# vpecanins/stm32f7-rtlsdr

Measured on AMD Instinct MI355X. Metric: IQ MSamples/s through FIR+FM-demod+resample, higher is better.
Workload: dtype f32 audio; K2 = u8 x 24-bit fixed-point taps on the i8 matrix pipe, exact i32 sums, one f32 recombination (design Q); K3 / K4 f32; ill-conditioned phases recomputed with the f32 fmaf chain

## Files before the change

stm32f7-rtlsdr_amd/csrc/sdrfm_q.hip:

```cpp
#include <hip/hip_runtime.h>
#include <hip/hip_ext.h>

#include <cstddef>
#include <cstdint>
#include <type_traits>

#include "sdrfm_math.h"
#include "sdrfm_q.h"
#include "sdrfm_b.h"

typedef int qi4_t __attribute__((ext_vector_type(4)));
typedef int qi8_t __attribute__((ext_vector_type(8)));
typedef float qf2_t __attribute__((ext_vector_type(2)));
__device__ void q_raw_buffer_load_lds(qi4_t rsrc, __attribute__((address_space(3))) void* lds, int size, int voffset, int soffset,
                                      int offset, int aux) __asm("llvm.amdgcn.raw.buffer.load.lds");

namespace {

constexpr int QTA = (int)SDRFM_Q_TA;
constexpr int DB0 = 128;
constexpr int ABS = 4;
constexpr int ABW = 128 * ABS;
constexpr int FLW = 64 + 2;
#ifndef SDRFM_Q_GTAB
// ... 4 lines not shown
constexpr int QTP = (int)SDRFM_Q_TP;
template <int D, int DA>
struct QGeo {
  static constexpr int NCH = D / 2;
  static constexpr int NSC = (D + 3) / 4;
  static constexpr int BLKB = 16 * D;
  static constexpr int STEPB = 16 * BLKB;
  static constexpr int PRE = BLKB;
  static constexpr int DBW = DB0 + 128 * DA + 16;
  static constexpr int RWIN = QTP + 2 * D;
  static constexpr bool ALIGNED = (STEPB % 1024) == 0;
  static constexpr int CS = STEPB / 1024;
  static_assert(QTP % 4 == 0 && (2 * D) % 4 == 0, "the repair path loads whole groups of four samples, none of which straddles the call's first sample");
  static_assert(QTP + 2 * D <= 96, "the tap table of the repair path sits below the d history");
  static_assert(D % 2 == 0 && D <= 16 && (ALIGNED || D == 10), "geometries the ring logic is written for");
};
#ifndef SDRFM_Q_HO_RING
#define SDRFM_Q_HO_RING 1
#endif
#ifndef SDRFM_Q_K3
#define SDRFM_Q_K3 1
#endif
#ifndef SDRFM_Q_XORSKIP
#define SDRFM_Q_XORSKIP 1
#endif
#ifndef SDRFM_Q_PEEL
#define SDRFM_Q_PEEL 1
#endif
#ifndef SDRFM_Q_MICRO
#define SDRFM_Q_MICRO 1
#endif
#ifndef SDRFM_Q_AUX
#define SDRFM_Q_AUX 2
#endif
#ifndef SDRFM_Q_WQB
#define SDRFM_Q_WQB 4
#endif
constexpr int WQB = SDRFM_Q_WQB;
static_assert(WQB >= 4 && WQB <= 16 && 8 * WQB >= (int)SDRFM_Q_TA, "a warm-up holds the d history of a run's first audio output");

__device__ __forceinline__ float q_discriminate(float yr, float yi, float pr, float pi) {
  const float re = __builtin_fmaf(yr, pr, yi * pi);
  const float im = yi * pr - yr * pi;
  const float ax = __builtin_fabsf(re), ay = __builtin_fabsf(im);
  const float mx = __builtin_fmaxf(__builtin_fmaxf(ax, ay), 0x1p-120f), mn = __builtin_fminf(ax, ay);
  const float v = mn * __builtin_amdgcn_rcpf(mx);
  const float s2 = v * v;
  float q = 0x1.e34882p-8f;
  q = __builtin_fmaf(q, s2, -0x1.22fc74p-5f);
  q = __builtin_fmaf(q, s2, 0x1.509024p-4f);
  q = __builtin_fmaf(q, s2, -0x1.12688cp-3f);
  q = __builtin_fmaf(q, s2, 0x1.96c562p-3f);
  q = __builtin_fmaf(q, s2, -0x1.554086p-2f);
  float a = __builtin_fmaf(v, s2 * q, v);
  if (ay > ax) a = 0x1.921fb6p+0f - a;
  if (re < 0.0f) a = 0x1.921fb6p+1f - a;
  return __builtin_copysignf(a, im);
}

__device__ __forceinline__ float q_angle(float yr, float yi, float& mx_out) {
  const float ax = __builtin_fabsf(yr), ay = __builtin_fabsf(yi);
  const float mx = __builtin_fmaxf(__builtin_fmaxf(ax, ay), 0x1p-120f), mn = __builtin_fminf(ax, ay);
  mx_out = mx;
  const float v = mn * __builtin_amdgcn_rcpf(mx);
  const float s2 = v * v;
  float q = 0x1.e34882p-8f;
  q = __builtin_fmaf(q, s2, -0x1.22fc74p-5f);
  q = __builtin_fmaf(q, s2, 0x1.509024p-4f);
  q = __builtin_fmaf(q, s2, -0x1.12688cp-3f);
  q = __builtin_fmaf(q, s2, 0x1.96c562p-3f);
  q = __builtin_fmaf(q, s2, -0x1.554086p-2f);
  float a = __builtin_fmaf(v, s2 * q, v);
  if (ay > ax) a = 0x1.921fb6p+0f - a;
  if (yr < 0.0f) a = 0x1.921fb6p+1f - a;
  return __builtin_copysignf(a, yi);
}
__device__ __forceinline__ float q_wrap(float x) {
  float t = __builtin_fmaf(x, 0x1.45f306p-3f, 0x1.8p+23f);
  asm volatile("" : "+v"(t));
  const float k = t - 0x1.8p+23f;
  return __builtin_fmaf(k, -0x1.921fb6p+2f, x);
}

__device__ __forceinline__ unsigned q_pcm_word(float v) {
  const float c = __builtin_amdgcn_fmed3f(v, -32768.0f, 32767.0f);
  float t = c + 0x1.8p+23f;
  asm volatile("" : "+v"(t));
  return __builtin_amdgcn_perm(__builtin_bit_cast(unsigned, t), __builtin_bit_cast(unsigned, t), 0x05040504u);
}

template <int N>
__device__ __forceinline__ void wait_vmcnt() {
  static_assert(N >= 0 && N < 16, "vmcnt immediate");
  __builtin_amdgcn_s_waitcnt(0x0f70 | N);
}

#ifdef SDRFM_Q_PHASES
#define Q_PHASE(i) do { const unsigned long long tn_ = __builtin_readcyclecounter(); t_ph[i] += tn_ - t_last; t_last = tn_; } while (0)
#else
#define Q_PHASE(i) do { } while (0)
#endif

template <int D, int DA, int NSLOT>
constexpr uint32_t q_lds() { return (uint32_t)(QGeo<D, DA>::PRE + 1024 * NSLOT + 4 * (QGeo<D, DA>::DBW + ABW + FLW + GTW)); }
struct QPcmArgs { SdrfmQParams p; SdrfmSinkChain t; };
static_assert(ABS * 128 <= 64 * (int)SDRFM_CHAIN_CH, "a flush of parked audio is one scan of the wave");
template <int C0, int NSLOT, int D, int DA, bool PCM = false>
__device__ __forceinline__ void mfir_body(const SdrfmQParams& p, const uint32_t bid) {
  using G = QGeo<D, DA>;
  [[maybe_unused]] constexpr int NCH = G::NCH;
  constexpr int QD = D, QDA = DA, NSC = G::NSC, BLKB = G::BLKB, STEPB = G::STEPB, PRE = G::PRE, DBW = G::DBW, RWIN = G::RWIN;
  constexpr bool ALIGNED = G::ALIGNED;
  constexpr int CS = G::CS;
  constexpr int RINGB = NSLOT * 1024;
  static_assert(RINGB % (2 * STEPB) == 0 && (ALIGNED ? NSLOT == 2 * CS : (NSLOT >= 5 && NSLOT - 4 < 16)), "ring: whole pairs of steps");
  extern __shared__ __attribute__((aligned(16))) unsigned char smem[];
  float* const db = reinterpret_cast<float*>(smem + PRE + RINGB);
  float* const ab = db + DBW;
  unsigned short* const fl16 = reinterpret_cast<unsigned short*>(ab + ABW);
  const int lane = (int)threadIdx.x, n = lane & 15, g = lane >> 4;
  const uint32_t si = bid / p.runs, run = bid - si * p.runs;
  const uint32_t stream = p.slist ? p.slist[si] : si;
  const uint32_t Bt = (p.M + 7u) >> 3, Qt = (Bt + WQB - 1u) / WQB, vs = p.iq_prev ? 1u : 0u;
  const uint32_t Gq = Qt + p.runs - 1u + vs;
  const uint32_t e0 = (uint32_t)(((uint64_t)run * Gq) / p.runs), e1 = (uint32_t)(((uint64_t)(run + 1) * Gq) / p.runs);
  const int q0 = run == 0 ? 0 : (int)e0 - (int)(run - 1u + vs), q1 = (int)e1 - (int)(run + vs);
  if (q0 >= q1) return;
  if (lane == 0) *reinterpret_cast<uint2*>(fl16 + 128) = make_uint2(0u, 0u);
#ifdef SDRFM_Q_STAMPS
  unsigned long long* const tsp = p.dbg ? p.dbg + 16 * (size_t)bid : nullptr;
  unsigned long long t_wait = 0, t_first = 0;
  const unsigned long long t_entry = __builtin_amdgcn_s_memrealtime();
  const unsigned long long c_entry = __builtin_readcyclecounter();
#endif
#ifdef SDRFM_Q_PHASES
  unsigned long long t_ph[8] = {0, 0, 0, 0, 0, 0, 0, 0}, t_last = 0;
#endif
  const bool from_prev = run == 0 && p.iq_prev != nullptr;
  const bool warm = run > 0 || from_prev;
  const int b0 = WQB * q0;
  int b1 = WQB * q1;
  if (b1 > (int)Bt) b1 = (int)Bt;
  const bool last_run = b1 == (int)Bt;
  const int bs = warm ? b0 - WQB : b0;
  const int nsteps = (b1 - bs + 15) >> 4;
  const int nlast = b1 - bs - 16 * (nsteps - 1);
  const int o0 = 8 * bs;
  const int jg0 = (o0 + 64 * QDA) / QDA - 64;
  const int jlo = warm ? (o0 + 8 * WQB) / QDA : 0;
  int j1 = (8 * b1) / QDA;
  if (j1 > (int)p.A_out) j1 = (int)p.A_out;
  const int phi = QDA * jg0 + QDA - 1 - o0;
  const int sigma = (phi + 1) & 1;

  float cr = 1.0e4f, ci = 0.0f;
  const int HT = (int)p.T - 1;
  unsigned short hb0 = 0, hb1 = 0;
  float hd0 = 0.0f;
  if (!warm) {
    const float2 yp = p.yprev_in[stream];
    cr = yp.x; ci = yp.y;
    const unsigned short* hbp = reinterpret_cast<const unsigned short*>(p.hist_b_in) + (size_t)stream * HT;
    if (lane < HT) hb0 = hbp[lane];
    if (lane + 64 < HT) hb1 = hbp[lane + 64];
    if (lane < QTA - 1) hd0 = p.hist_d_in[(size_t)stream * (QTA - 1) + lane];
  }

  const unsigned long long gaddr = (unsigned long long)(p.iq + (size_t)stream * p.iq_stride);
  uint32_t hi = (uint32_t)BLKB * (uint32_t)b1;
  if (hi > 2u * p.N) hi = 2u * p.N;
  const qi4_t rsrc = {(int)(unsigned)gaddr, (int)(unsigned)(gaddr >> 32), (int)hi, 0x00020000};
  const int lsw0 = ALIGNED ? ((16 * lane) ^ (((((16 * lane) / BLKB)) & 7) << 4)) : 16 * lane;
  const int lsw1 = ALIGNED ? ((16 * lane) ^ (((((1024 + 16 * lane) / BLKB)) & 7) << 4)) : 16 * lane;
  const int gb = BLKB * bs;
  int vpos = gb + (ALIGNED ? 0 : 16 * lane);
  auto slot_ptr = [&](int slot) { return (__attribute__((address_space(3))) void*)(smem + PRE + 1024 * slot); };
  auto lsw = [&](int chunk) { return (BLKB == 256 && (chunk & 1)) ? lsw1 : lsw0; };
  constexpr int HL = BLKB / 16, HK = ALIGNED ? 7 : 0;
  const unsigned long long pa = from_prev ? (unsigned long long)(p.iq_prev + (size_t)stream * p.iq_prev_stride) + 2ull * p.N_prev - (WQB + 1) * BLKB : 0ull;
  const qi4_t rprev = {(int)(unsigned)pa, (int)(unsigned)(pa >> 32), (WQB + 1) * BLKB, 0x00020000};
  if (warm && lane < HL) {
    const int hv = 16 * (lane ^ HK);
    if (from_prev) q_raw_buffer_load_lds(rprev, (__attribute__((address_space(3))) void*)smem, 16, hv, 0, 0, SDRFM_Q_AUX);
    else q_raw_buffer_load_lds(rsrc, (__attribute__((address_space(3))) void*)smem, 16, gb - BLKB + hv, 0, 0, SDRFM_Q_AUX);
  }
  if constexpr (ALIGNED) {
#pragma unroll
    for (int q = 0; q < CS; ++q) {
      const int off = gb + 1024 * q + lsw(q);
      if (from_prev && off < 0) q_raw_buffer_load_lds(rprev, slot_ptr(q), 16, off + (WQB + 1) * BLKB, 0, 0, SDRFM_Q_AUX);
      else q_raw_buffer_load_lds(rsrc, slot_ptr(q), 16, off, 0, 0, SDRFM_Q_AUX);
    }
  } else {
    auto first_step_chunk = [&](int c, __attribute__((address_space(3))) void* lds, int imm) {
      const int off = vpos + 1024 * c;
      if (from_prev && off < 0) q_raw_buffer_load_lds(rprev, lds, 16, off - imm + (WQB + 1) * BLKB, 0, imm, SDRFM_Q_AUX);
      else q_raw_buffer_load_lds(rsrc, lds, 16, off - imm, 0, imm, SDRFM_Q_AUX);
    };
    first_step_chunk(0, slot_ptr(0), 0);
    first_step_chunk(1, slot_ptr(1), 0);
    first_step_chunk(2, slot_ptr(0), 2048);
  }
  __builtin_amdgcn_sched_barrier(0);
  asm volatile("" ::: "memory");
  qi4_t At[NSC - C0][SDRFM_Q_DIGITS];
#pragma unroll
  for (int c = C0; c < NSC; ++c)
#pragma unroll
    for (int t = 0; t < SDRFM_Q_DIGITS; ++t)
#if defined(SDRFM_Q_ABLATE) && (SDRFM_Q_ABLATE & 4)
      At[c - C0][t] = qi4_t{lane + c, lane * t, c - t, lane};
// ... 77 lines not shown
    const unsigned long long tw0 = __builtin_readcyclecounter();
#endif
#ifdef SDRFM_Q_FIRSTWAIT
    if (!ALIGNED && first) wait_vmcnt<(ALIGNED ? CS : NSLOT - 3)>();
    else
#endif
    wait_vmcnt<(ALIGNED ? CS : NSLOT - 4)>();
    asm volatile("" ::: "memory");
#ifdef SDRFM_Q_LDSXOR
#pragma unroll
    for (int i = 0; i < STEPB / 512; ++i)
      (void)__hip_atomic_fetch_xor(reinterpret_cast<unsigned long long*>(__builtin_assume_aligned(smem + PRE + ringoff + 8 * (lane + 64 * i), 8)), 0x8080808080808080ull, __ATOMIC_RELAXED, __HIP_MEMORY_SCOPE_WAVEFRONT);
#endif
#ifdef SDRFM_Q_STAMPS
    t_wait += __builtin_readcyclecounter() - tw0;
    if (t_first == 0) t_first = __builtin_amdgcn_s_memrealtime();
#endif
    if constexpr (ALIGNED) {
      const int ro0 = n == 0 ? 0 : ringoff;
#pragma unroll
      for (int c = 2 * C0; c < 2 * NSC; ++c) dst[c - 2 * C0] = *reinterpret_cast<const qi4_t*>(smem + rdoff[c] + (64 * c < BLKB ? ro0 : ringoff));
      if (lane < BLKB / 16) {
        const qi4_t hcp = *reinterpret_cast<const qi4_t*>(smem + PRE + ringoff + STEPB - BLKB + 16 * lane);
        *reinterpret_cast<qi4_t*>(smem + 16 * lane) = hcp;
      }
      __builtin_amdgcn_wave_barrier();
    } else {
      const unsigned char* wb = smem + baddr + ringoff;
#pragma unroll
      for (int c = 2 * C0; c < 2 * NSC; ++c) dst[c - 2 * C0] = *reinterpret_cast<const qi4_t*>(wb + 64 * c);
      if (ringoff + STEPB == RINGB) {
        if (lane < BLKB / 16) {
          const qi4_t hcp = *reinterpret_cast<const qi4_t*>(smem + PRE + RINGB - BLKB + 16 * lane);
          *reinterpret_cast<qi4_t*>(smem + 16 * lane) = hcp;
        }
        __builtin_amdgcn_wave_barrier();
      }
    }
    if constexpr (RINGB == 2 * STEPB) ringoff ^= STEPB;
    else ringoff = (ringoff + STEPB == RINGB) ? 0 : ringoff + STEPB;
  };
  auto refill_step = [&](int k) {
    asm volatile("s_waitcnt lgkmcnt(0)" ::: "memory");
    if constexpr (ALIGNED) {
#pragma unroll
      for (int q = 0; q < CS; ++q) q_raw_buffer_load_lds(rsrc, slot_ptr(slot + q), 16, vpos + 1024 * q + lsw(q), 0, 0, SDRFM_Q_AUX);
      slot = slot ? 0 : CS;
      vpos += STEPB;
      return;
    }
    if constexpr (NSLOT == 5 && SDRFM_Q_PEEL) {
      if (k & 1) {
        q_raw_buffer_load_lds(rsrc, slot_ptr(2), 16, vpos, 0, 0, SDRFM_Q_AUX);
        q_raw_buffer_load_lds(rsrc, slot_ptr(2), 16, vpos, 0, 1024, SDRFM_Q_AUX);
        vpos += 2048;
      } else {
        if (k > 0) {
          q_raw_buffer_load_lds(rsrc, slot_ptr(4), 16, vpos, 0, 0, SDRFM_Q_AUX);
          vpos += 1024;
        }
        q_raw_buffer_load_lds(rsrc, slot_ptr(0), 16, vpos, 0, 0, SDRFM_Q_AUX);
        q_raw_buffer_load_lds(rsrc, slot_ptr(0), 16, vpos, 0, 1024, SDRFM_Q_AUX);
        vpos += 2048;
      }
      return;
    }
    if (k > 0 && !(k & 1)) {
      q_raw_buffer_load_lds(rsrc, slot_ptr(slot), 16, vpos, 0, 0, SDRFM_Q_AUX);
      vpos += 1024;
      slot = (slot + 1 == NSLOT) ? 0 : slot + 1;
    }
    q_raw_buffer_load_lds(rsrc, slot_ptr(slot), 16, vpos, 0, 0, SDRFM_Q_AUX);
    q_raw_buffer_load_lds(rsrc, slot_ptr(slot), 16, vpos, 0, 1024, SDRFM_Q_AUX);
    slot = (slot + 2 >= NSLOT) ? slot + 2 - NSLOT : slot + 2;
    vpos += 2048;
  };
  typedef const __attribute__((address_space(4))) SdrfmQParams* KargPtr;
  auto kargs = [&]() -> KargPtr {
    KargPtr pp = (KargPtr)__builtin_amdgcn_kernarg_segment_ptr();
    asm volatile("" : "+s"(pp));
    return pp;
  };
  int npend = 0, jfl = jg0;
  [[maybe_unused]] float yrun = 0.0f;
  [[maybe_unused]] bool pfirst = true;
  [[maybe_unused]] float* const pstash = reinterpret_cast<float*>(smem + q_lds<D, DA, NSLOT>());
  typedef const __attribute__((address_space(4))) SdrfmSinkChain* KChainPtr;
  [[maybe_unused]] auto kchain = [&]() -> KChainPtr {
    const __attribute__((address_space(4))) unsigned char* pp = (const __attribute__((address_space(4))) unsigned char*)__builtin_amdgcn_kernarg_segment_ptr();
    asm volatile("" : "+s"(pp));
    return (KChainPtr)(pp + offsetof(QPcmArgs, t));
  };
  [[maybe_unused]] unsigned long long pv_early = 0ull;
  [[maybe_unused]] bool published = false;
  [[maybe_unused]] float dp_early = 0.0f;
  auto flush_audio = [&](const bool fin = false) {
    __builtin_amdgcn_wave_barrier();
#if defined(SDRFM_Q_ABLATE) && (SDRFM_Q_ABLATE & 256)
    float* row = p.audio - jfl;
    const int ln_ = lane;
#else
    uint32_t st_ = stream;
    int ln_ = lane;
    asm volatile("" : "+s"(st_), "+v"(ln_));
    float* row = kargs()->audio + (size_t)st_ * kargs()->audio_stride;
#endif
    const int lo = jfl > jlo ? jfl : jlo;
#if defined(SDRFM_Q_ABLATE) && (SDRFM_Q_ABLATE & 128)
    const int hi_ = (ab[lane] == 1234.5f) ? lo + 2 : lo;
#else
    const int hi_ = (j1 < jfl + 128 * npend) ? j1 : jfl + 128 * npend;
#endif
    const int par = (int)((reinterpret_cast<uintptr_t>(row) >> 2) & 1u);
    bool want_audio = true;
    if constexpr (PCM) want_audio = kargs()->audio != nullptr;
    if (want_audio) for (int e = lo - ((lo + par) & 1) + 2 * ln_; e < hi_; e += 128) {
      const bool v0 = e >= lo, v1 = e + 1 < hi_;
      const float a0 = v0 ? ab[e - jfl] : 0.0f, a1 = v1 ? ab[e + 1 - jfl] : 0.0f;
      if constexpr (PCM) {
        if (v0 && v1) __builtin_nontemporal_store(qf2_t{a0, a1}, reinterpret_cast<qf2_t*>(row + e));
        else if (v0) __builtin_nontemporal_store(a0, row + e);
        else if (v1) __builtin_nontemporal_store(a1, row + e + 1);
      } else {
        if (v0 && v1) *reinterpret_cast<qf2_t*>(row + e) = qf2_t{a0, a1};
        else if (v0) row[e] = a0;
        else if (v1) row[e + 1] = a1;
      }
    }
    if constexpr (PCM) {
      const int cntf = hi_ - lo;
      if (cntf > 0) {
        constexpr int PCH = (int)SDRFM_CHAIN_CH, FIX = (int)SDRFM_CHAIN_FIX;
        const KChainPtr tp = kchain();
        const float alpha = tp->alpha, gain = tp->gain;
        asm volatile("s_waitcnt lgkmcnt(0)" ::: "memory");
        __builtin_amdgcn_wave_barrier();
        float* const xa = ab + (lo - jfl);
        unsigned* const xw = reinterpret_cast<unsigned*>(xa);
        const int i0 = PCH * ln_;
        float xr[PCH];
#pragma unroll
        for (int q = 0; q < PCH; ++q) xr[q] = (i0 + q < cntf) ? xa[i0 + q] : 0.0f;
        float sc = 0.0f;
#pragma unroll
        for (int q = 0; q < PCH; ++q) sc = __builtin_fmaf(tp->w[q], xr[q], sc);
        float pw = tp->pc;
        if (ln_ == 0) sc = __builtin_fmaf(pw, yrun, sc);
#pragma unroll
        for (int d = 1; d < 64; d <<= 1) {
          const float o = __shfl_up(sc, (unsigned)d, 64);
          const float sn = __builtin_fmaf(pw, o, sc);
          sc = ln_ >= d ? sn : sc;
          pw *= pw;
        }
        if (fin) {
          const int Ll = (cntf - 1) / PCH, rl = (cntf - 1) % PCH;
          const float ypub = __shfl(sc, Ll, 64) * tp->dinv[PCH - 1 - rl];
          uint32_t bid2 = bid;
          asm volatile("" : "+s"(bid2));
          if (ln_ == 0) {
            const uint32_t call = tp->call, nst = tp->n_streams;
            const unsigned long long w = ((unsigned long long)((last_run ? call : tp->run_call) + 1u) << 32) | __builtin_bit_cast(unsigned, ypub);
            __hip_atomic_store(last_run ? tp->sg + (size_t)((call + 1u) % SDRFM_CHAIN_SG_SLOTS) * nst + st_ : tp->runstate + bid2, w, __ATOMIC_RELAXED,
                               __HIP_MEMORY_SCOPE_AGENT);
            unsigned long long zero = 0ull;
            asm volatile("" : "+v"(zero));
            pv_early = __hip_atomic_fetch_add(run == 0 ? tp->sg + (size_t)(call % SDRFM_CHAIN_SG_SLOTS) * nst + st_ : tp->runstate + (bid2 - 1u), zero,
                                              __ATOMIC_RELAXED, __HIP_MEMORY_SCOPE_AGENT);
          }
          dp_early = ln_ < (int)SDRFM_CHAIN_FIX ? tp->dpow[ln_] : 0.0f;
          published = true;
        }
        float y = __shfl_up(sc, 1u, 64);
        if (ln_ == 0) y = yrun;
        __builtin_amdgcn_wave_barrier();
#pragma unroll
        for (int q = 0; q < PCH; ++q) {
          const float yn = __builtin_fmaf(alpha, xr[q] - y, y);
          y = (i0 + q < cntf) ? yn : y;
          if (i0 + q < cntf) {
            xw[i0 + q] = q_pcm_word(yn * gain);
            if (pfirst && i0 + q < FIX) pstash[i0 + q] = yn;
          }
        }
        yrun = __shfl(y, (cntf - 1) / PCH, 64);
        __builtin_amdgcn_wave_barrier();
        unsigned* const out = reinterpret_cast<unsigned*>(tp->pcm + (size_t)st_ * tp->pcm_stride);
        const int parp = (int)((reinterpret_cast<uintptr_t>(out) >> 2) & 1u), ps = lo + (pfirst ? FIX : 0);
        for (int e = ps - ((ps + parp) & 1) + 2 * ln_; e < hi_; e += 128) {
          const bool v0 = e >= ps, v1 = e + 1 < hi_;
          const unsigned w0 = v0 ? xw[e - lo] : 0u, w1 = v1 ? xw[e + 1 - lo] : 0u;
          if (v0 && v1) *reinterpret_cast<uint2*>(out + e) = make_uint2(w0, w1);
          else if (v0) out[e] = w0;
          else if (v1) out[e + 1] = w1;
        }
        pfirst = false;
      }
    }
    jfl += 128 * npend;
    npend = 0;
  };
  int nflag = 0;
  auto repair_flagged = [&]() {
    int ln = lane;
    uint32_t st = stream;
    asm volatile("" : "+v"(ln), "+s"(st));
    const KargPtr pp = kargs();
#ifdef SDRFM_Q_PHASES
    unsigned long long r_t0 = __builtin_readcyclecounter(), r_t1;
#define R_PHASE(word, shift, waitfirst) do { if (waitfirst) asm volatile("s_waitcnt vmcnt(0) lgkmcnt(0)" ::: "memory"); r_t1 = __builtin_readcyclecounter(); \
                                             t_ph[word] += ((r_t1 - r_t0) & 0xffffffffull) << shift; r_t0 = r_t1; } while (0)
#else
#define R_PHASE(word, shift, waitfirst) do { } while (0)
#endif
    const unsigned char* const row = pp->iq + (size_t)st * pp->iq_stride;
    const unsigned char* const pre = from_prev ? pp->iq_prev + (size_t)st * pp->iq_prev_stride + 2 * (size_t)pp->N_prev
                                               : pp->hist_q_in + (size_t)(2 * QTP) * ((size_t)st + 1);
    unsigned* const cnt = reinterpret_cast<unsigned*>(fl16 + 128);
    __builtin_amdgcn_wave_barrier();
    unsigned nrep = 0;
    for (int e0 = 0; e0 < nflag; e0 += 64) {
      const int e = e0 + ln;
      int l = 0, slot = 0, m0 = (int)pp->M;
      if (e < nflag) {
        const unsigned ent = fl16[e];
        l = (int)(ent & 63u);
        slot = (int)(ent >> 6) - 1;
        m0 = mbase + 128 * slot + 8 * (l & 15) + 2 * (l >> 4);
      }
      const bool act = m0 < (int)pp->M;
      nrep += (unsigned)__builtin_popcountll(__builtin_amdgcn_ballot_w64(act));
      if (act) {
        const int n0 = QD * m0 - QTP;
        uint2 w[RWIN / 4];
#pragma unroll
        for (int c = 0; c < RWIN / 4; ++c) {
          const int n = n0 + 4 * c;
          w[c] = *reinterpret_cast<const uint2*>((n >= 0 ? row : pre) + 2 * (ptrdiff_t)n);
        }
        R_PHASE(0, 0, 0);
        R_PHASE(0, 32, 1);
        qf2_t a[3] = {qf2_t{0.0f, 0.0f}, qf2_t{0.0f, 0.0f}, qf2_t{0.0f, 0.0f}};
        const float* const hz = db;
#pragma unroll
        for (int i = 0; i < RWIN; ++i) {
          const unsigned wd = (i & 2) ? w[i >> 2].y : w[i >> 2].x;
          const qf2_t b = {(float)((wd >> ((i & 1) ? 16 : 0)) & 0xffu), (float)((wd >> ((i & 1) ? 24 : 8)) & 0xffu)};
          const qf2_t x = b - qf2_t{127.5f, 127.5f};
#pragma unroll
          for (int o = 0; o < 3; ++o) {
            const int u = i - QD * o + 2 * QD;
            if (u < 2 * QD || u >= QTP + 2 * QD) continue;
            const float t = hz[u];
            a[o] = __builtin_elementwise_fma(qf2_t{t, t}, x, a[o]);
          }
          if ((i & 7) == 7) __builtin_amdgcn_sched_barrier(0);
        }
        if (m0 == 0 && !warm && pp->yprev_exact) {
          const float2 yp = pp->yprev_in[st];
          a[0] = qf2_t{yp.x, yp.y};
        }
        float* dst = db + DB0 + sigma + 128 * slot + 8 * (l & 15) + 2 * (l >> 4);
        dst[0] = sdrfm_discriminate(a[1].x, a[1].y, a[0].x, a[0].y);
        dst[1] = sdrfm_discriminate(a[2].x, a[2].y, a[1].x, a[1].y);
      }
    }
    R_PHASE(7, 0, 1);
    if (ln == 0) {
      cnt[0] += nrep;
      cnt[1] += 1u;
    }
    nflag = 0;
    R_PHASE(7, 32, 1);
  };
#ifdef SDRFM_Q_GUARD_L1
  float guard_r = 2.0f * p.guard_r, guard_a = p.guard_a;
#else
  float guard_r = p.guard_r, guard_a = p.guard_a;
#endif
  asm volatile("" : "+v"(guard_r), "+v"(guard_a));
// ... 184 lines not shown
    }
    __builtin_amdgcn_wave_barrier();
    if (LAST && last_run && lane < QTA - 1) {
      const KargPtr pp = kargs();
      pp->hist_d_out[(size_t)stream * (QTA - 1) + lane] = db[DB0 + sigma + ((int)pp->M - (QTA - 1) + lane - mbase)];
    }
#ifdef SDRFM_Q_PHASES
    asm volatile("s_waitcnt lgkmcnt(0)" ::: "memory");
#endif
    Q_PHASE(5);

    if (osm == QDA || (LAST && osm > 0)) {
      const float* w = db + DB0 + sigma + phi + 2 * QDA * lane - (QTA - 1);
      float dw[QTA + QDA + 3];
#pragma unroll
      for (int i = 0; i < (QTA + QDA + 3) / 2; ++i) {
        const qf2_t v = *reinterpret_cast<const qf2_t*>(w + 2 * i);
        dw[2 * i] = v.x;
        dw[2 * i + 1] = v.y;
      }
      float a0 = 0.0f, a0b = 0.0f, a1 = 0.0f, a1b = 0.0f;
#if SDRFM_Q_GTAB
#pragma unroll
      for (int q = 0; q < QTA / 8; ++q) {
        const qf4_t tl = *reinterpret_cast<const qf4_t*>(gt + 4 * q), th = *reinterpret_cast<const qf4_t*>(gt + QTA / 2 + 4 * q);
#pragma unroll
        for (int i = 0; i < 4; ++i) {
          const int k = 4 * q + i;
          a0 = __builtin_fmaf(tl[i], dw[k], a0);
          a0b = __builtin_fmaf(th[i], dw[QTA / 2 + k], a0b);
          a1 = __builtin_fmaf(tl[i], dw[QDA + k], a1);
          a1b = __builtin_fmaf(th[i], dw[QDA + QTA / 2 + k], a1b);
        }
      }
#else
#pragma unroll
      for (int k = 0; k < QTA / 2; ++k) {
        a0 = __builtin_fmaf(gr[k], dw[k], a0);
        a0b = __builtin_fmaf(gr[QTA / 2 + k], dw[QTA / 2 + k], a0b);
        a1 = __builtin_fmaf(gr[k], dw[QDA + k], a1);
        a1b = __builtin_fmaf(gr[QTA / 2 + k], dw[QDA + QTA / 2 + k], a1b);
      }
#endif
      a0 += a0b;
      a1 += a1b;
      *reinterpret_cast<qf2_t*>(ab + 128 * npend + 2 * lane) = qf2_t{a0, a1};
      ++npend;
      if (osm == QDA) {
        if (lane < QTA) {
          const float hv = db[DB0 + sigma + 128 * QDA - QTA + lane];
          db[DB0 + sigma - QTA + lane] = hv;
        }
        __builtin_amdgcn_wave_barrier();
        osm = 0;
        mbase += 128 * QDA;
      }
      if (npend == ABS) flush_audio();
      Q_PHASE(6);
    }
#if SDRFM_Q_PEEL
  };
  for (int kk = 0; kk < nsteps - 1; ++kk) step(std::false_type{}, kk);
  step(std::true_type{}, nsteps - 1);
#else
  }
#endif
#ifdef SDRFM_Q_STAMPS
  const unsigned long long t_loop = __builtin_amdgcn_s_memrealtime();
#endif
  wait_vmcnt<0>();
  flush_audio(true);
  if constexpr (PCM) {
    const KChainPtr tp = kchain();
    uint32_t st_ = stream, bid_ = bid;
    int ln_ = lane;
    asm volatile("" : "+s"(st_), "+s"(bid_), "+v"(ln_));
    const uint32_t call = tp->call, nst = tp->n_streams;
    unsigned long long* const rs = tp->runstate;
    unsigned long long* const sg = tp->sg;
    const float dp = published ? dp_early : (ln_ < (int)SDRFM_CHAIN_FIX ? tp->dpow[ln_] : 0.0f);
    unsigned long long pv = pv_early;
    if (ln_ == 0) {
      if (!published) {
        const unsigned long long w = ((unsigned long long)((last_run ? call : tp->run_call) + 1u) << 32) | __builtin_bit_cast(unsigned, yrun);
        __hip_atomic_store(last_run ? sg + (size_t)((call + 1u) % SDRFM_CHAIN_SG_SLOTS) * nst + st_ : rs + bid_, w, __ATOMIC_RELAXED, __HIP_MEMORY_SCOPE_AGENT);
      }
      unsigned long long* const src = run == 0 ? sg + (size_t)(call % SDRFM_CHAIN_SG_SLOTS) * nst + st_ : rs + (bid_ - 1u);
      const uint32_t want = run == 0 ? call : tp->run_call + 1u;
      unsigned long long zero = 0ull;
      asm volatile("" : "+v"(zero));
      int it = 0;
      for (;; ++it) {
        if (it > 0 || !published) pv = __hip_atomic_fetch_add(src, zero, __ATOMIC_RELAXED, __HIP_MEMORY_SCOPE_AGENT);
        if ((uint32_t)(pv >> 32) == want || it == (1 << 19)) break;
        __builtin_amdgcn_s_sleep(16);
      }
      if (it == (1 << 19)) { pv = 0ull; __hip_atomic_store(tp->err, 1u, __ATOMIC_RELAXED, __HIP_MEMORY_SCOPE_AGENT); }
    }
    const float carry = __builtin_bit_cast(float, __builtin_amdgcn_readfirstlane((int)(unsigned)pv));
    const int nfix = (j1 - jlo < (int)SDRFM_CHAIN_FIX) ? j1 - jlo : (int)SDRFM_CHAIN_FIX;
    if (ln_ < nfix) {
      const float yv = __builtin_fmaf(dp, carry, pstash[ln_]);
      reinterpret_cast<unsigned*>(tp->pcm + (size_t)st_ * tp->pcm_stride)[jlo + ln_] = q_pcm_word(yv * tp->gain);
    }
  }
  const KargPtr pe = kargs();
  if (pe->n_repaired && lane == 0) {
    const uint2 cnt = *reinterpret_cast<const uint2*>(fl16 + 128);
    if (cnt.y) {
      atomicAdd(pe->n_repaired, cnt.x);
      atomicAdd(pe->n_repaired + 1, cnt.y);
      if (pe->stream_pass) atomicAdd(pe->stream_pass + stream, cnt.y);
    }
  }

  if (last_run && !(SDRFM_Q_HO_RING && !ALIGNED)) {
    const unsigned char* row = pe->iq + (size_t)stream * pe->iq_stride;
    const int HTe = (int)pe->T - 1;
    const size_t Ne = pe->N;
    for (int k = lane; k < HTe; k += 64) {
      const unsigned raw = *reinterpret_cast<const unsigned short*>(row + 2 * (Ne - HTe + k));
      reinterpret_cast<unsigned short*>(pe->hist_b_out)[(size_t)stream * HTe + k] = (unsigned short)raw;
      pe->hist_x_out[(size_t)stream * HTe + k] = make_float2((float)(raw & 0xffu) - 127.5f, (float)(raw >> 8) - 127.5f);
    }
    if (lane < 2 * QTP / 16)
      *reinterpret_cast<qi4_t*>(pe->hist_q_out + (size_t)(2 * QTP) * stream + 16 * lane) =
          *reinterpret_cast<const qi4_t*>(row + 2 * Ne - 2 * QTP + 16 * lane);
  }
#ifdef SDRFM_Q_STAMPS
  if (tsp && lane == 0) {
    tsp[0] = t_entry; tsp[1] = t_first; tsp[2] = t_loop; tsp[3] = __builtin_amdgcn_s_memrealtime(); tsp[4] = t_wait;
#ifdef SDRFM_Q_PHASES
    for (int i = 0; i < 8; ++i) tsp[8 + i] = t_ph[i];
#endif
    tsp[5] = (__builtin_amdgcn_s_getreg((3 << 11) | 20) & 7) | ((unsigned long long)__builtin_amdgcn_s_getreg((31 << 11) | 4) << 8);
    tsp[6] = (unsigned long long)nsteps; tsp[7] = __builtin_readcyclecounter() - c_entry;
  }
#endif
}


template <int C0, int NSLOT, int D, int DA>
__global__ void __launch_bounds__(64) __attribute__((amdgpu_waves_per_eu(D == 16 ? 3 : 4))) k_mfir(SdrfmQParams p) {
  mfir_body<C0, NSLOT, D, DA>(p, blockIdx.x);
}

template <int C0, int NSLOT, int D, int DA>
__global__ void __launch_bounds__(64) __attribute__((amdgpu_waves_per_eu(D == 16 ? 3 : 4))) k_mfir_pcm(QPcmArgs a) {
  mfir_body<C0, NSLOT, D, DA, true>(a.p, blockIdx.x);
}

template <int C0, int NSLOT, int D, int DA, int T, int R>
__global__ void __launch_bounds__(64) __attribute__((amdgpu_waves_per_eu(3, 4))) k_mix(SdrfmQParams q, CallParams b, uint32_t nb) {
  if (blockIdx.x < nb) fastb_body<T, D, R, (int)SDRFM_Q_TA, DA, 0>(b, blockIdx.x);
  else mfir_body<C0, NSLOT, D, DA>(q, blockIdx.x - nb);
}

struct MixPcmArgs { QPcmArgs qa; CallParams b; uint32_t nb; };
template <int C0, int NSLOT, int D, int DA, int T, int R>
__global__ void __launch_bounds__(64) __attribute__((amdgpu_waves_per_eu(3, 4))) k_mix_pcm(MixPcmArgs a) {
  if (blockIdx.x < a.nb) fastb_body<T, D, R, (int)SDRFM_Q_TA, DA, 0>(a.b, blockIdx.x);
  else mfir_body<C0, NSLOT, D, DA, true>(a.qa.p, blockIdx.x - a.nb);
}

__global__ void __launch_bounds__(64) k_q_fix_yprev(const uint8_t* hist_q, const float* hpad, float2* yprev, uint32_t n_streams, const uint32_t* list) {
  const uint32_t i = blockIdx.x * 64 + threadIdx.x;
  if (i >= n_streams) return;
  const uint32_t s = list ? list[i] : i;
  const uint8_t* b = hist_q + (size_t)(2 * QTP) * s;
  float ar = 0.0f, ai = 0.0f;
  for (int i = 0; i < QTP; ++i) {
    const float t = hpad[QTP - 1 - i];
    ar = __builtin_fmaf(t, (float)b[2 * i] - 127.5f, ar);
    ai = __builtin_fmaf(t, (float)b[2 * i + 1] - 127.5f, ai);
  }
  yprev[s] = make_float2(ar, ai);
}

template <int NSLOT>
__global__ void __launch_bounds__(64) k_q_read_stream(const uint8_t* base, unsigned total_kib, unsigned kib_per_wave, unsigned* sink) {
  extern __shared__ __attribute__((aligned(16))) unsigned char smem[];
  const unsigned w = blockIdx.x, lane = threadIdx.x;
  const unsigned long long ga = (unsigned long long)base + ((unsigned long long)w * kib_per_wave << 10);
  const unsigned left = total_kib > w * kib_per_wave ? total_kib - w * kib_per_wave : 0u;
  const unsigned mine = left < kib_per_wave ? left : kib_per_wave;
  const qi4_t rsrc = {(int)(unsigned)ga, (int)(unsigned)(ga >> 32), (int)(mine << 10), 0x00020000};
// ... 171 lines not shown
```

Measured before the change: 2.524 million.

## Store PCM words from registers with aligned vector runs and keep carry state in LDS

In the PCM path, the flush now writes the packed PCM words straight from registers. Each lane's run of eight words goes out as aligned 4-wide and 2-wide vector stores, with cross-lane permutes to handle misalignment, instead of being written back to LDS and re-read in 2-wide strided stores. The running IIR state moves from a register to an LDS word, several wave barriers and lgkmcnt waits are dropped, shuffles become explicit bpermute/readlane, and the final fix-up words are written as paired stores. The aim is fewer LDS round trips, syncs and store instructions in the audio/PCM epilogue, at the cost of much more complex alignment and edge handling.

```diff
diff --git a/stm32f7-rtlsdr_amd/csrc/sdrfm_q.hip b/stm32f7-rtlsdr_amd/csrc/sdrfm_q.hip
--- a/stm32f7-rtlsdr_amd/csrc/sdrfm_q.hip
+++ b/stm32f7-rtlsdr_amd/csrc/sdrfm_q.hip
@@ -110,11 +110,87 @@
   return __builtin_fmaf(k, -0x1.921fb6p+2f, x);
 }
 
-__device__ __forceinline__ unsigned q_pcm_word(float v) {
-  const float c = __builtin_amdgcn_fmed3f(v, -32768.0f, 32767.0f);
+struct QPcmConsts { float lo, hi; unsigned sel; };
+__device__ __forceinline__ QPcmConsts q_pcm_consts() {
+  QPcmConsts c = {-32768.0f, 32767.0f, 0x05040504u};
+  asm volatile("" : "+v"(c.lo), "+v"(c.hi), "+s"(c.sel));
+  return c;
+}
+__device__ __forceinline__ unsigned q_pcm_word(float v, const QPcmConsts& k) {
+  const float c = __builtin_amdgcn_fmed3f(v, k.lo, k.hi);
   float t = c + 0x1.8p+23f;
   asm volatile("" : "+v"(t));
-  return __builtin_amdgcn_perm(__builtin_bit_cast(unsigned, t), __builtin_bit_cast(unsigned, t), 0x05040504u);
+  return __builtin_amdgcn_perm(__builtin_bit_cast(unsigned, t), __builtin_bit_cast(unsigned, t), k.sel);
+}
+
+template <bool NT, typename E>
+__device__ __forceinline__ void q_store_run8(E* const base, const E (&v)[8], const int kfirst, const int cnt, const int ln) {
+  static_assert(sizeof(E) == 4, "row elements are words");
+  typedef E V2 __attribute__((ext_vector_type(2)));
+  typedef E V4 __attribute__((ext_vector_type(4)));
+  auto st1 = [](E* p, E a) { if constexpr (NT) __builtin_nontemporal_store(a, p); else *p = a; };
+  auto st2 = [](E* p, E a, E b) { const V2 t = {a, b}; if constexpr (NT) __builtin_nontemporal_store(t, reinterpret_cast<V2*>(p)); else *reinterpret_cast<V2*>(p) = t; };
+  auto st4 = [](E* p, E a, E b, E c, E d) { const V4 t = {a, b, c, d}; if constexpr (NT) __builtin_nontemporal_store(t, reinterpret_cast<V4*>(p)); else *reinterpret_cast<V4*>(p) = t; };
+  const int s = (int)((0u - (unsigned)(reinterpret_cast<uintptr_t>(base) >> 2)) & 3u);
+  E nx[3] = {v[0], v[1], v[2]};
+  if (s != 0) {
+#pragma unroll
+    for (int j = 0; j < 3; ++j)
+      nx[j] = __builtin_bit_cast(E, __builtin_amdgcn_ds_bpermute(4 * ln + 4, __builtin_bit_cast(int, v[j])));
+  }
+  const int k0 = 8 * ln;
+  if (k0 < kfirst) return;
+  auto pieces = [&](auto S_) {
+    constexpr int S = decltype(S_)::value;
+    if (S > 0 && k0 == kfirst) {
+      if constexpr ((S & 1) != 0) { if (k0 < cnt) st1(base + k0, v[0]); }
+      if constexpr ((S & 2) != 0) {
+        constexpr int j = S & 1;
+        if (k0 + j + 1 < cnt) st2(base + k0 + j, v[j], v[j + 1]);
+        else if (k0 + j < cnt) st1(base + k0 + j, v[j]);
+      }
+    }
+    const E e[11] = {v[0], v[1], v[2], v[3], v[4], v[5], v[6], v[7], nx[0], nx[1], nx[2]};
+#pragma unroll
+    for (int p = 0; p < 2; ++p) {
+      const int kp = k0 + S + 4 * p, nleft = cnt - kp;
+      const E a = e[S + 4 * p], b = e[S + 4 * p + 1], c = e[S + 4 * p + 2], d = e[S + 4 * p + 3];
+      if (nleft >= 4) st4(base + kp, a, b, c, d);
+      else if (nleft > 0) {
+        if (nleft >= 2) st2(base + kp, a, b);
+        if (nleft & 1) st1(base + kp + (nleft & 2), (nleft & 2) ? c : a);
+      }
+    }
+  };
+  switch (s) {
+    case 0: pieces(std::integral_constant<int, 0>{}); break;
+    case 1: pieces(std::integral_constant<int, 1>{}); break;
+    case 2: pieces(std::integral_constant<int, 2>{}); break;
+    default: pieces(std::integral_constant<int, 3>{}); break;
+  }
+}
+
+template <bool NT, typename E>
+__device__ __forceinline__ void q_store_lying(E* const base, const E* const src, const int kfirst, const int cnt, const int ln) {
+  typedef E V2 __attribute__((ext_vector_type(2)));
+  const int par = (int)((reinterpret_cast<uintptr_t>(base) >> 2) & 1u);
+  const int kb = kfirst - ((kfirst + par) & 1) + 2 * ln;
+#pragma unroll
+  for (int it = 0; it <= ABS; ++it) {
+    const int k = kb + 128 * it;
+    if (k >= cnt) break;
+    const bool v0 = k >= kfirst, v1 = k + 1 < cnt;
+    const E a0 = v0 ? src[k] : E(0), a1 = v1 ? src[k + 1] : E(0);
+    if constexpr (NT) {
+      if (v0 && v1) __builtin_nontemporal_store(V2{a0, a1}, reinterpret_cast<V2*>(base + k));
+      else if (v0) __builtin_nontemporal_store(a0, base + k);
+      else if (v1) __builtin_nontemporal_store(a1, base + k + 1);
+    } else {
+      if (v0 && v1) *reinterpret_cast<V2*>(base + k) = V2{a0, a1};
+      else if (v0) base[k] = a0;
+      else if (v1) base[k + 1] = a1;
+    }
+  }
 }
 
 template <int N>
@@ -155,6 +231,10 @@
   const int q0 = run == 0 ? 0 : (int)e0 - (int)(run - 1u + vs), q1 = (int)e1 - (int)(run + vs);
   if (q0 >= q1) return;
   if (lane == 0) *reinterpret_cast<uint2*>(fl16 + 128) = make_uint2(0u, 0u);
+  if constexpr (PCM) {
+    static_assert(SDRFM_Q_GTAB == 1, "the two words between the repair list's counters and the audio taps");
+    if (lane == 0) reinterpret_cast<float*>(fl16)[FLW] = 0.0f;
+  }
 #ifdef SDRFM_Q_STAMPS
   unsigned long long* const tsp = p.dbg ? p.dbg + 16 * (size_t)bid : nullptr;
   unsigned long long t_wait = 0, t_first = 0;
@@ -398,8 +478,7 @@
     return pp;
   };
   int npend = 0, jfl = jg0;
-  [[maybe_unused]] float yrun = 0.0f;
-  [[maybe_unused]] bool pfirst = true;
+  [[maybe_unused]] float* const yrunp = reinterpret_cast<float*>(fl16) + FLW;
   [[maybe_unused]] float* const pstash = reinterpret_cast<float*>(smem + q_lds<D, DA, NSLOT>());
   typedef const __attribute__((address_space(4))) SdrfmSinkChain* KChainPtr;
   [[maybe_unused]] auto kchain = [&]() -> KChainPtr {
@@ -412,51 +491,28 @@
   [[maybe_unused]] float dp_early = 0.0f;
   auto flush_audio = [&](const bool fin = false) {
     __builtin_amdgcn_wave_barrier();
-#if defined(SDRFM_Q_ABLATE) && (SDRFM_Q_ABLATE & 256)
-    float* row = p.audio - jfl;
-    const int ln_ = lane;
-#else
-    uint32_t st_ = stream;
-    int ln_ = lane;
-    asm volatile("" : "+s"(st_), "+v"(ln_));
-    float* row = kargs()->audio + (size_t)st_ * kargs()->audio_stride;
-#endif
-    const int lo = jfl > jlo ? jfl : jlo;
-#if defined(SDRFM_Q_ABLATE) && (SDRFM_Q_ABLATE & 128)
-    const int hi_ = (ab[lane] == 1234.5f) ? lo + 2 : lo;
-#else
-    const int hi_ = (j1 < jfl + 128 * npend) ? j1 : jfl + 128 * npend;
-#endif
-    const int par = (int)((reinterpret_cast<uintptr_t>(row) >> 2) & 1u);
-    bool want_audio = true;
-    if constexpr (PCM) want_audio = kargs()->audio != nullptr;
-    if (want_audio) for (int e = lo - ((lo + par) & 1) + 2 * ln_; e < hi_; e += 128) {
-      const bool v0 = e >= lo, v1 = e + 1 < hi_;
-      const float a0 = v0 ? ab[e - jfl] : 0.0f, a1 = v1 ? ab[e + 1 - jfl] : 0.0f;
-      if constexpr (PCM) {
-        if (v0 && v1) __builtin_nontemporal_store(qf2_t{a0, a1}, reinterpret_cast<qf2_t*>(row + e));
-        else if (v0) __builtin_nontemporal_store(a0, row + e);
-        else if (v1) __builtin_nontemporal_store(a1, row + e + 1);
-      } else {
-        if (v0 && v1) *reinterpret_cast<qf2_t*>(row + e) = qf2_t{a0, a1};
-        else if (v0) row[e] = a0;
-        else if (v1) row[e + 1] = a1;
-      }
-    }
     if constexpr (PCM) {
+      constexpr int PCH = (int)SDRFM_CHAIN_CH, FIX = (int)SDRFM_CHAIN_FIX;
+      const int lo = jfl > jlo ? jfl : jlo;
+      const int hi_ = (j1 < jfl + 128 * npend) ? j1 : jfl + 128 * npend;
       const int cntf = hi_ - lo;
       if (cntf > 0) {
-        constexpr int PCH = (int)SDRFM_CHAIN_CH, FIX = (int)SDRFM_CHAIN_FIX;
+        uint32_t st_ = stream;
+        int ln_ = lane;
+        asm volatile("" : "+s"(st_), "+v"(ln_));
+        const bool first = jfl <= jlo;
         const KChainPtr tp = kchain();
         const float alpha = tp->alpha, gain = tp->gain;
-        asm volatile("s_waitcnt lgkmcnt(0)" ::: "memory");
-        __builtin_amdgcn_wave_barrier();
-        float* const xa = ab + (lo - jfl);
-        unsigned* const xw = reinterpret_cast<unsigned*>(xa);
-        const int i0 = PCH * ln_;
+        const float* const xa = ab + (lo - jfl);
+        const int i0 = PCH * ln_, nv = cntf - i0;
         float xr[PCH];
 #pragma unroll
-        for (int q = 0; q < PCH; ++q) xr[q] = (i0 + q < cntf) ? xa[i0 + q] : 0.0f;
+        for (int q = 0; q < PCH; ++q) xr[q] = (q < nv) ? xa[i0 + q] : 0.0f;
+        float* const arow = kargs()->audio;
+        if (arow) q_store_lying<true>(arow + (size_t)st_ * kargs()->audio_stride + lo, xa, 0, cntf, ln_);
+        const float yrun = *yrunp;
+        auto lane_up = [&](float v, int d) { return __builtin_bit_cast(float, __builtin_amdgcn_ds_bpermute(4 * (ln_ - d), __builtin_bit_cast(int, v))); };
+        auto lane_of = [&](float v, int l) { return __builtin_bit_cast(float, __builtin_amdgcn_readlane(__builtin_bit_cast(int, v), l)); };
         float sc = 0.0f;
 #pragma unroll
         for (int q = 0; q < PCH; ++q) sc = __builtin_fmaf(tp->w[q], xr[q], sc);
@@ -464,14 +520,14 @@
         if (ln_ == 0) sc = __builtin_fmaf(pw, yrun, sc);
 #pragma unroll
         for (int d = 1; d < 64; d <<= 1) {
-          const float o = __shfl_up(sc, (unsigned)d, 64);
+          const float o = lane_up(sc, d);
           const float sn = __builtin_fmaf(pw, o, sc);
           sc = ln_ >= d ? sn : sc;
           pw *= pw;
         }
         if (fin) {
           const int Ll = (cntf - 1) / PCH, rl = (cntf - 1) % PCH;
-          const float ypub = __shfl(sc, Ll, 64) * tp->dinv[PCH - 1 - rl];
+          const float ypub = lane_of(sc, Ll) * tp->dinv[PCH - 1 - rl];
           uint32_t bid2 = bid;
           asm volatile("" : "+s"(bid2));
           if (ln_ == 0) {
@@ -487,31 +543,49 @@
           dp_early = ln_ < (int)SDRFM_CHAIN_FIX ? tp->dpow[ln_] : 0.0f;
           published = true;
         }
-        float y = __shfl_up(sc, 1u, 64);
+        float y = lane_up(sc, 1);
         if (ln_ == 0) y = yrun;
-        __builtin_amdgcn_wave_barrier();
+        unsigned xw[PCH];
+        const QPcmConsts kc = q_pcm_consts();
 #pragma unroll
         for (int q = 0; q < PCH; ++q) {
           const float yn = __builtin_fmaf(alpha, xr[q] - y, y);
-          y = (i0 + q < cntf) ? yn : y;
-          if (i0 + q < cntf) {
-            xw[i0 + q] = q_pcm_word(yn * gain);
-            if (pfirst && i0 + q < FIX) pstash[i0 + q] = yn;
-          }
+          y = (q < nv) ? yn : y;
+          xw[q] = q_pcm_word(yn * gain, kc);
+          if (first && ln_ < FIX / PCH && q < nv) pstash[i0 + q] = yn;
         }
-        yrun = __shfl(y, (cntf - 1) / PCH, 64);
-        __builtin_amdgcn_wave_barrier();
-        unsigned* const out = reinterpret_cast<unsigned*>(tp->pcm + (size_t)st_ * tp->pcm_stride);
-        const int parp = (int)((reinterpret_cast<uintptr_t>(out) >> 2) & 1u), ps = lo + (pfirst ? FIX : 0);
-        for (int e = ps - ((ps + parp) & 1) + 2 * ln_; e < hi_; e += 128) {
-          const bool v0 = e >= ps, v1 = e + 1 < hi_;
-          const unsigned w0 = v0 ? xw[e - lo] : 0u, w1 = v1 ? xw[e + 1 - lo] : 0u;
-          if (v0 && v1) *reinterpret_cast<uint2*>(out + e) = make_uint2(w0, w1);
-          else if (v0) out[e] = w0;
-          else if (v1) out[e + 1] = w1;
+        if (!fin) {
+          const float yend = lane_of(y, (cntf - 1) / PCH);
+          if (ln_ == 0) *yrunp = yend;
         }
-        pfirst = false;
-      }
+        q_store_run8<false>(reinterpret_cast<unsigned*>(tp->pcm + (size_t)st_ * tp->pcm_stride) + lo, xw, first ? FIX : 0, cntf, ln_);
+      }
+      jfl += 128 * npend;
+      npend = 0;
+      return;
+    }
+#if defined(SDRFM_Q_ABLATE) && (SDRFM_Q_ABLATE & 256)
+    float* row = p.audio - jfl;
+    const int ln_ = lane;
+#else
+    uint32_t st_ = stream;
+    int ln_ = lane;
+    asm volatile("" : "+s"(st_), "+v"(ln_));
+    float* row = kargs()->audio + (size_t)st_ * kargs()->audio_stride;
+#endif
+    const int lo = jfl > jlo ? jfl : jlo;
+#if defined(SDRFM_Q_ABLATE) && (SDRFM_Q_ABLATE & 128)
+    const int hi_ = (ab[lane] == 1234.5f) ? lo + 2 : lo;
+#else
+    const int hi_ = (j1 < jfl + 128 * npend) ? j1 : jfl + 128 * npend;
+#endif
+    const int par = (int)((reinterpret_cast<uintptr_t>(row) >> 2) & 1u);
+    for (int e = lo - ((lo + par) & 1) + 2 * ln_; e < hi_; e += 128) {
+      const bool v0 = e >= lo, v1 = e + 1 < hi_;
+      const float a0 = v0 ? ab[e - jfl] : 0.0f, a1 = v1 ? ab[e + 1 - jfl] : 0.0f;
+      if (v0 && v1) *reinterpret_cast<qf2_t*>(row + e) = qf2_t{a0, a1};
+      else if (v0) row[e] = a0;
+      else if (v1) row[e + 1] = a1;
     }
     jfl += 128 * npend;
     npend = 0;
@@ -862,7 +936,7 @@
     unsigned long long pv = pv_early;
     if (ln_ == 0) {
       if (!published) {
-        const unsigned long long w = ((unsigned long long)((last_run ? call : tp->run_call) + 1u) << 32) | __builtin_bit_cast(unsigned, yrun);
+        const unsigned long long w = ((unsigned long long)((last_run ? call : tp->run_call) + 1u) << 32) | __builtin_bit_cast(unsigned, *yrunp);
         __hip_atomic_store(last_run ? sg + (size_t)((call + 1u) % SDRFM_CHAIN_SG_SLOTS) * nst + st_ : rs + bid_, w, __ATOMIC_RELAXED, __HIP_MEMORY_SCOPE_AGENT);
       }
       unsigned long long* const src = run == 0 ? sg + (size_t)(call % SDRFM_CHAIN_SG_SLOTS) * nst + st_ : rs + (bid_ - 1u);
@@ -879,9 +953,17 @@
     }
     const float carry = __builtin_bit_cast(float, __builtin_amdgcn_readfirstlane((int)(unsigned)pv));
     const int nfix = (j1 - jlo < (int)SDRFM_CHAIN_FIX) ? j1 - jlo : (int)SDRFM_CHAIN_FIX;
+    unsigned* const out = reinterpret_cast<unsigned*>(tp->pcm + (size_t)st_ * tp->pcm_stride) + jlo;
+    const float yv = __builtin_fmaf(dp, carry, ln_ < nfix ? pstash[ln_] : 0.0f);
+    const unsigned wd = q_pcm_word(yv * tp->gain, q_pcm_consts());
+    const unsigned wn = (unsigned)__builtin_amdgcn_ds_bpermute(4 * ln_ + 4, (int)wd);
     if (ln_ < nfix) {
-      const float yv = __builtin_fmaf(dp, carry, pstash[ln_]);
-      reinterpret_cast<unsigned*>(tp->pcm + (size_t)st_ * tp->pcm_stride)[jlo + ln_] = q_pcm_word(yv * tp->gain);
+      if ((((unsigned)(reinterpret_cast<uintptr_t>(out) >> 2) + (unsigned)ln_) & 1u) == 0u) {
+        if (ln_ + 1 < nfix) *reinterpret_cast<uint2*>(out + ln_) = make_uint2(wd, wn);
+        else out[ln_] = wd;
+      } else if (ln_ == 0) {
+        out[0] = wd;
+      }
     }
   }
   const KargPtr pe = kargs();
```

After: 2.513 million. No clear change (-0.4%).
